# TGoldC/Motion-Planning-for-Autonomous-Driving-with-MPC

Hardware: AMD Instinct MI355X
Metric: MPC steps/sec (N=30, nx=6 nu=2) at batch=4096 (higher is better)
Workload: dtype f64; 1 GPU; N=30 nx=6 nu=2 bicycle lane-following, batch=4096/GPU, tol 1e-8; mode=converged, gpu=AMD Radeon Graphics

## Files before the change

### motion-planning-for-autonomous-driving-with-mpc_amd/csrc/mpc_solve_plan.h

```cpp
#pragma once
#include <algorithm>
#include <cctype>
#include <cstdlib>
#include <cstring>
#include <string>

#include "mpc_host_common.h"

namespace mpc {

struct Knobs {
    int pipeline, hybrid, hybrid_bx, hybrid_live, pipe_help, pipe_test_abort, pipe_xcd_mask;
    int rescue, rescue_wg, rescue_alone, loop_async, sync_spin, max_batch, friction_lb, bound_mask, big_wg, groups, poison;
    int timing;
    Knobs();
};
enum class KnobParse {
    ON,
    INT,
    FLAG,
    MASK,
    FRIC,
};
struct KnobDef { const char* name; int Knobs::*field; int dflt; KnobParse parse; };
inline constexpr KnobDef KNOBS[] = {
    {"pipeline", &Knobs::pipeline, 1, KnobParse::ON},           {"hybrid", &Knobs::hybrid, 1, KnobParse::INT},
    {"hybrid_bx", &Knobs::hybrid_bx, 0, KnobParse::INT},        {"hybrid_live", &Knobs::hybrid_live, -1, KnobParse::INT},
    {"pipe_help", &Knobs::pipe_help, -1, KnobParse::INT},       {"pipe_test_abort", &Knobs::pipe_test_abort, 0, KnobParse::FLAG},
    {"pipe_xcd_mask", &Knobs::pipe_xcd_mask, 0, KnobParse::MASK}, {"rescue", &Knobs::rescue, 1, KnobParse::ON},
    {"rescue_wg", &Knobs::rescue_wg, 1, KnobParse::INT},        {"rescue_alone", &Knobs::rescue_alone, 0, KnobParse::FLAG},
    {"loop_async", &Knobs::loop_async, 1, KnobParse::ON},       {"sync_spin", &Knobs::sync_spin, 1, KnobParse::ON},
    {"max_batch", &Knobs::max_batch, 0, KnobParse::INT},        {"friction_lb", &Knobs::friction_lb, 0, KnobParse::FRIC},
    {"bound_mask", &Knobs::bound_mask, 1, KnobParse::INT},      {"big_wg", &Knobs::big_wg, 0, KnobParse::FLAG},
    {"groups", &Knobs::groups, 0, KnobParse::INT},              {"poison", &Knobs::poison, 0, KnobParse::FLAG},
    {"timing", &Knobs::timing, 0, KnobParse::INT},
};
inline Knobs::Knobs() { for (const KnobDef& e : KNOBS) this->*e.field = e.dflt; }
inline const KnobDef* find_knob(const char* name) {
    for (const KnobDef& e : KNOBS) if (name && strcmp(name, e.name) == 0) return &e;
    return nullptr;
}
inline int set_knob(Knobs& k, const char* name, const char* value) {
    const KnobDef* e = find_knob(name);
    if (!e) return MPC_ERR_INVALID;
    int v = e->dflt;
    if (value) {
        const long iv = strtol(value, nullptr, 0);
        switch (e->parse) {
            case KnobParse::ON: v = value[0] != '0'; break;
            case KnobParse::INT: v = (int)iv; break;
            case KnobParse::FLAG: v = (value[0] == '\0' ? 1 : (int)iv) != 0; break;
            case KnobParse::MASK: v = (int)(uint32_t)strtoul(value, nullptr, 0); break;
            case KnobParse::FRIC: v = strcmp(value, "ipopt") == 0 ? 1 : strcmp(value, "nlp") == 0 ? 0 : (int)iv; break;
        }
    }
    k.*e->field = v;
    return MPC_OK;
}
// ... 19 lines not shown
              TIMING_WG_TRACE = 16;

constexpr int STAGE_MAX_THREADS = 512;
constexpr int MAX_GROUPS = 4;
constexpr int MAX_POLL_IT = 1024;
constexpr size_t LDS_MAX = 160 * 1024 - 1024;

#ifndef MPC_STAGE_STASH
#define MPC_STAGE_STASH 1
#endif
template <int NX> struct Stash {
    static constexpr int rows(bool has_ou) { return 4 * (NX + 2) + 2 * 3 + (has_ou ? 2 * 3 : 0) + 3 + 2 * NX; }
};

constexpr uint32_t REF_BOUND_VM = 0x33u;
constexpr uint32_t REF_DENSE_LO = 0x31u, REF_DENSE_HI = 0x33u;

constexpr int RIC_DEPTH = 4;
constexpr int RIC_DEPTH_F = 10;

constexpr uint32_t PIPE_X_STRIDE = 64;
enum PipeXcdWord : uint32_t { PX_ARRIVE = 0, PX_HEAD = 16, PX_TAIL = 32, PX_FINISHED = 48, PX_HO_TICKET = 56 };
constexpr uint32_t PIPE_ABORT = 8 * PIPE_X_STRIDE;
constexpr uint32_t HO_BUCKETS = 4;
enum PipeHeadWord : uint32_t {
    PH_ABORT = 0, PH_ROUNDS = 1,
    PH_STAT64 = 2,
    PH_STAGE_WORKERS = 12, PH_RIC_WORKERS = 13, PH_FAIL = 14,
    PH_WG = 16,
    PH_HELPED = 21, PH_FIN_TICKET = 22,
    PH_HO = 24,
    PH_DETAIL = 28,
    PH_WORDS = 32 };
enum PipeStat64 : uint32_t { P64_RIC_WAIT, P64_STAGE_WAIT, P64_STAGE_BUSY, P64_ITEMS };
enum WgStatWord : uint32_t { WGS_ROUNDS_MAX, WGS_ROUNDS, WGS_SWEEPS, WGS_INST_ROUNDS, WGS_RESCUED, WGS_WORDS };
constexpr uint32_t PIPE_STATS = PIPE_ABORT + PH_STAT64, PIPE_WG = PIPE_ABORT + PH_WG, PIPE_HO = PIPE_ABORT + PH_HO, PIPE_HDR = PIPE_ABORT + PH_WORDS;
struct CtlField { uint32_t at, words, align; };
template <size_t N> constexpr bool ctl_fields_ok(const CtlField (&f)[N], uint32_t size) {
    for (size_t i = 0; i < N; ++i) {
        if (f[i].at % f[i].align || f[i].at + f[i].words > size) return false;
        for (size_t j = 0; j < i; ++j) if (f[i].at < f[j].at + f[j].words && f[j].at < f[i].at + f[i].words) return false;
    }
    return true;
}
constexpr CtlField PIPE_HEAD_FIELDS[] = {{PH_ABORT, 1, 1}, {PH_ROUNDS, 1, 1}, {PH_STAT64, 8, 2}, {PH_STAGE_WORKERS, 1, 1}, {PH_RIC_WORKERS, 1, 1}, {PH_FAIL, 1, 1},
                                         {PH_WG, WGS_WORDS, 1}, {PH_HELPED, 1, 1}, {PH_FIN_TICKET, 1, 1}, {PH_HO, HO_BUCKETS, 1}, {PH_DETAIL, 4, 1}};
constexpr CtlField PIPE_XCD_FIELDS[] = {{PX_ARRIVE, 1, 1}, {PX_HEAD, 1, 1}, {PX_TAIL, 1, 1}, {PX_FINISHED, 1, 1}, {PX_HO_TICKET, 1, 1}};
static_assert(ctl_fields_ok(PIPE_HEAD_FIELDS, PH_WORDS) && PIPE_ABORT % 2 == 0 && PH_HO + HO_BUCKETS <= PH_DETAIL, "the head's fields are disjoint, inside it, the uint64 ones 8-byte aligned; the hand-over counters end in front of the abort details");
static_assert(ctl_fields_ok(PIPE_XCD_FIELDS, PIPE_X_STRIDE), "the fields of an XCD record are disjoint and inside it");
constexpr uint32_t pipe_slots_off(uint32_t ntiles) { return (PIPE_HDR + ntiles + 1u) & ~1u; }
constexpr size_t pipe_ctl_words(uint32_t ntiles, uint32_t cap) { return (size_t)pipe_slots_off(ntiles) + (size_t)16 * cap; }
constexpr int PIPE_MAX_TILES = 256;

constexpr size_t prestart_doubles(int NX, int S, int bx) { return (size_t)4 * S * (NX + 2) + (size_t)(3 * NX + 2) * S * bx + (size_t)4 * bx; }
template <int NX>
struct WgLds {
    static constexpr int PAD = Rec<NX>::SIZE > 64 ? Rec<NX>::SIZE : 64;
    static constexpr size_t doubles(int S, int bxw) { return (size_t)PAD + (size_t)Rec<NX>::SIZE * S * bxw + (size_t)2 * S * (NX + 2) + (size_t)16 * bxw + (size_t)64 * NX + (size_t)WgScl::SIZE * bxw; }
};

struct PlanState {
    int n_cu = 256;
    uint32_t xcd_mask = 0xFFu;
    bool ws_mailbox = false;
    bool pipe_disabled = false;
    bool resc_hint = false;
    int32_t B = 0;
    bool per_inst_obst = false;
    bool trace = false;
    bool in_rescue = false;
    bool async_loop = false;
};
struct SolvePlan {
    bool small_wg;
    int S, bx, threads, nblk, ntiles, G, stash_rows;
    size_t lds_bytes, lds_init, ric_lds;
    bool masked;
    int cap, chunk;
    bool polled;
    bool fused;
    size_t lds_pre, lds_start;
    bool res_path, pipe_path;
    int hyb_bx;
    bool resc_alone, hyb_ok;
    int hand;
    bool wg_resc;
    size_t wg_lds;
    int wg_grid;
    uint32_t xcd_mask;
    int n_xcd, tiles_x, cu_x, n_ric;
    uint32_t pipe_cap;
    bool pipe_help;
    int mbw_live;
    bool stage_timing, start_timing, wg_timing, wg_trace, pipe_timing, poison;
    size_t max_rows;
    bool mailbox;
    bool rescue;
    bool loop_async;
};

template <int NX>
SolvePlan plan_solve_nx(const HostProblem& hp, const Knobs& kn, const PlanState& st) {
    const mpc_problem_desc& d = hp.desc;
    const int B = st.B;
    SolvePlan pl{};
    const size_t Bp = ((size_t)B + 63) / 64 * 64;
    const int S = d.N + 1;
    pl.S = S;
    pl.ntiles = (int)(Bp / 64);
    const int ntiles = pl.ntiles;
    pl.small_wg = 4 * S <= 256 && !kn.big_wg;
// ... 24 lines not shown
    pl.fused = lds_red + pl.lds_pre + 16 + lds_in <= 78 * 1024 && d.N >= 1 && pl.small_wg;
    pl.lds_start = std::max(lds_red + pl.lds_pre + 16 + lds_in, pl.lds_init);

    auto wg_lds = [&](int bxw) {
        const size_t pre = prestart_doubles(NX, S, bxw) * sizeof(double);
        const size_t init = ((size_t)10 * bxw + (size_t)2 * S * (NX + 2) + (size_t)2 * NX * 64) * sizeof(double);
        return std::max(WgLds<NX>::doubles(S, bxw) * sizeof(double), bxw == 1 ? std::max(pre, init) : (size_t)0);
    };
    pl.rescue = kn.rescue && d.fixed_iters <= 0 && !st.trace && hp.has_ol && hp.ol_raw > 0.0;
    const bool resc_cond = pl.rescue && (kn.rescue_wg >= 2 || kn.rescue_alone || (kn.rescue_wg == 1 && st.resc_hint)) && !st.in_rescue;
    int hyb_bx = ((kn.hybrid_bx == 2 || (kn.hybrid_bx == 0 && B > 4 * st.n_cu)) && S * 2 <= 64) ? 2 : 1;
    if (kn.hybrid_bx == 0 && resc_cond && hyb_bx == 2 && (size_t)ntiles * 64 * 8 <= (size_t)4 * st.n_cu * 18) hyb_bx = 1;
    pl.resc_alone = kn.rescue_alone && kn.hybrid_bx == 0 && kn.hybrid_live < 0 && resc_cond && ntiles <= 128;
    if (pl.resc_alone || st.in_rescue) hyb_bx = 1;
    pl.hyb_bx = hyb_bx;
    pl.wg_resc = resc_cond && hyb_bx == 1;
    pl.wg_lds = wg_lds(hyb_bx);
    pl.mailbox = pl.small_wg && S <= 64 && kn.hybrid && d.fixed_iters <= 0 && kn.pipeline && !st.pipe_disabled;
    pl.hyb_ok = kn.hybrid && st.ws_mailbox && d.fixed_iters <= 0 && kn.pipeline && !st.pipe_disabled && G == 1 && pl.small_wg && S <= 64 &&
                pl.wg_lds <= LDS_MAX / 4 && !st.trace && !pl.stage_timing;
    int hand = 0;
    if (pl.hyb_ok) {
        const int base = std::min(64, 4 * st.n_cu * hyb_bx / std::max(1, ntiles));
        hand = base >= 64 ? base : std::max(base, std::min(50, base < 32 ? 7 * base / 4 : 3 * base / 2));
        if (hyb_bx == 1 && base < 64 && hand < 40) hand = 40;
        if ((size_t)ntiles * 64 * 8 <= (size_t)4 * st.n_cu * hyb_bx * (hyb_bx == 2 ? 9 : 18)) hand = 64;
        if (pl.resc_alone) hand = 64;
        if (kn.hybrid_live >= 0) hand = std::min(64, kn.hybrid_live);
    }
    pl.hand = hand;
    pl.res_path = pl.hyb_ok && (hand >= 64 || st.in_rescue);
    pl.xcd_mask = st.xcd_mask;
    if (kn.pipe_xcd_mask) {
        const uint32_t m = (uint32_t)kn.pipe_xcd_mask & st.xcd_mask;
        if (m) pl.xcd_mask = m;
    }
    pl.n_xcd = __builtin_popcount(pl.xcd_mask);
    pl.tiles_x = (ntiles + pl.n_xcd - 1) / pl.n_xcd;
    pl.cu_x = std::max(2, st.n_cu / pl.n_xcd);
    const int tiles_x = pl.tiles_x, cu_x = pl.cu_x;
    const int n_ric_base = std::max(1, cu_x / 4);
    const bool ric_per_tile = tiles_x > n_ric_base && tiles_x <= 3 * cu_x / 8 && (64 / bx) * tiles_x <= 5 * (cu_x - tiles_x) && S >= 24;
    pl.n_ric = std::min(ric_per_tile ? tiles_x : n_ric_base, tiles_x);
    const bool eligible = G == 1 && !st.trace && !pl.stage_timing && pl.small_wg && pl.threads >= 192 && pl.threads <= 256 &&
                          ntiles <= (d.fixed_iters > 0 ? 64 : PIPE_MAX_TILES) && (tiles_x + pl.n_ric - 1) / pl.n_ric <= 32 &&
                          std::max(pl.lds_bytes, pl.ric_lds) <= LDS_MAX;
    pl.pipe_path = !pl.res_path && eligible && !st.pipe_disabled && kn.pipeline;
    pl.pipe_cap = 1;
    while (pl.pipe_path && pl.pipe_cap < 2u * (64u / (uint32_t)bx) * (uint32_t)tiles_x) pl.pipe_cap <<= 1;
    pl.pipe_help = pl.pipe_path && pl.masked && (kn.pipe_help < 0 ? (64 / bx) * tiles_x > 3 * (cu_x - pl.n_ric) : kn.pipe_help != 0);
    pl.mbw_live = pl.pipe_path && hand > 0 ? std::min(63, hand + 16) : 0;
    pl.wg_grid = pl.res_path ? (B + hyb_bx - 1) / hyb_bx
               : pl.pipe_path && hand > 0 ? std::min((B + hyb_bx - 1) / hyb_bx, std::max(4 * st.n_cu, (int)((size_t)hand * ntiles + hyb_bx - 1) / hyb_bx)) : 0;
    pl.start_timing = (kn.timing & TIMING_START) && !st.async_loop && G == 1;
    pl.wg_timing = (kn.timing & TIMING_WG) && !st.async_loop;
    pl.wg_trace = (kn.timing & TIMING_WG_TRACE) && !st.async_loop && !st.in_rescue;
    pl.pipe_timing = (kn.timing & TIMING_PIPE) != 0;
    pl.poison = kn.poison && !st.in_rescue;

    const WsLayout w1 = ws_layout(d.N, NX, 64, pl.mailbox);
    pl.max_rows = (((size_t)1 << 32) - 1) / (w1.total * sizeof(double)) * 64;
    const bool pipe_shape = pl.small_wg && kn.pipeline && !st.pipe_disabled && kn.groups <= 0 && !pl.stage_timing && d.fixed_iters <= 0 &&
                            pl.threads >= 192 && pl.threads <= 256;
    if (pipe_shape) pl.max_rows = std::min(pl.max_rows, (size_t)PIPE_MAX_TILES * 64);
    if (kn.max_batch > 0) pl.max_rows = std::min(pl.max_rows, (size_t)(kn.max_batch + 63) / 64 * 64);
    pl.loop_async = d.fixed_iters <= 0 && kn.pipeline && !st.pipe_disabled && kn.loop_async && (size_t)B <= pl.max_rows;
    return pl;
}
inline SolvePlan plan_solve(const HostProblem& hp, const Knobs& kn, const PlanState& st) {
    return hp.desc.nx == 5 ? plan_solve_nx<5>(hp, kn, st) : plan_solve_nx<6>(hp, kn, st);
}

struct SolveIo {
    int32_t B = 0;
    const double *x0 = nullptr, *p = nullptr, *obst = nullptr;
    double *x_out = nullptr, *kkt = nullptr;
// ... 18 lines not shown
```

### motion-planning-for-autonomous-driving-with-mpc_amd/csrc/mpcgpu.hip

```cpp
#include <hip/hip_runtime.h>
#include <type_traits>

#include <algorithm>
#include <cctype>
#include <cstdio>
#include <cstdlib>
#include <cstring>
#include <new>
#include <string>
#include <vector>

#include "mpc_host_common.h"
#include "mpc_solve_plan.h"
#include "mpc_stamps.h"
#include "mpc_closed_loop.h"
#include "mpc_forces_qp.h"
#include "mpc_riccati_mfma.h"
#include "mpc_sens.h"

using namespace mpc;

namespace {

__device__ __forceinline__ void lds_barrier() {
// ... 280 lines not shown
    const uint32_t b0 = (blk + (uint32_t)P.tile0 * (64u / (uint32_t)P.bx)) * (uint32_t)P.bx;
    const unsigned long long bits = (!INIT && P.tile_mask != nullptr) ? P.tile_mask[b0 >> 6] : ~0ull;
    stage_block<NX, INIT, MAXT, VM>(P, n_mult, n_z, stash_rows, b0, bits, lds);
}

constexpr int32_t HO_IN_MB = 0x40000000;

template <int NCH>
__device__ __forceinline__ void wait_dma_behind(int stages_behind) {
    if (stages_behind >= 4 && 4 * NCH <= 63) asm volatile("s_waitcnt vmcnt(%0)" ::"n"(4 * NCH <= 63 ? 4 * NCH : 0) : "memory");
    else if (stages_behind >= 3 && 3 * NCH <= 63) asm volatile("s_waitcnt vmcnt(%0)" ::"n"(3 * NCH <= 63 ? 3 * NCH : 0) : "memory");
    else if (stages_behind >= 2) asm volatile("s_waitcnt vmcnt(%0)" ::"n"(2 * NCH) : "memory");
    else if (stages_behind == 1) asm volatile("s_waitcnt vmcnt(%0)" ::"n"(NCH) : "memory");
    else asm volatile("s_waitcnt vmcnt(0)" ::: "memory");
}

__device__ __forceinline__ void ho_lists(const PRef& P, const uint32_t bb, int32_t* ho_list, uint32_t* ho_count, const uint32_t* tile_word) {
#if defined(__HIP_DEVICE_COMPILE__)
    const int lane = threadIdx.x & 63;
    const bool active = (int)bb < P.B && (int32_t)MPC_U(P.ISC, (uint32_t)IS_STATUS) == ST_RUNNING;
    if (__ballot(active ? 1 : 0) == 0ull) return;
    const int32_t in_mb = (tile_word != nullptr && (__hip_atomic_load(tile_word + (bb >> 6), __ATOMIC_RELAXED, __HIP_MEMORY_SCOPE_AGENT) >> 31)) ? HO_IN_MB : 0;
    const double e0 = active ? (double)MPC_U(P.SC, (uint32_t)SC_E0) : 0.0;
    const int bucket = e0 >= 1e-3 ? 0 : e0 >= 1e-4 ? 1 : e0 >= 1e-5 ? 2 : 3;
    for (int q = 0; q < (int)HO_BUCKETS; ++q) {
        const unsigned long long mq = __ballot((active && bucket == q) ? 1 : 0);
        if (mq == 0ull) continue;
        uint32_t base = 0u;
        if (lane == 0) base = __hip_atomic_fetch_add(ho_count + q, (uint32_t)__popcll(mq), __ATOMIC_RELAXED, __HIP_MEMORY_SCOPE_AGENT);
        base = (uint32_t)__builtin_amdgcn_readfirstlane((int)base);
        if (active && bucket == q) ho_list[(uint32_t)q * (uint32_t)P.Bp + base + (uint32_t)__popcll(mq & ((1ull << lane) - 1ull))] = (int32_t)bb | in_mb;
    }
#endif
}

template <int NX>
__device__ __forceinline__ unsigned long long riccati_tile(const PRef& P, const uint32_t tile, char* smem, const bool stamp = true, const int handover_live = 0) {
#if defined(__HIP_DEVICE_COMPILE__)
    using D = Dim<NX>;
    constexpr int NS = D::NS;
    constexpr uint32_t BLK_BYTES = MPC_EV(D::NBLK) * 512u;
    constexpr int BLK_CHUNKS = (BLK_BYTES + 1023u) / 1024u;
    constexpr uint32_t SLOT = BLK_CHUNKS * 1024u;
    constexpr int KK_CHUNKS = (D::NKK * 512u + 1023u) / 1024u;
    constexpr int FWD_CHUNKS = KK_CHUNKS + 6;
    constexpr uint32_t FSLOT = FWD_CHUNKS * 1024u;
    static_assert(2 * BLK_CHUNKS <= 63 && RIC_DEPTH == 4 && 4 * FWD_CHUNKS <= 63 && RIC_DEPTH_F == 10, "vmcnt is a 6-bit counter");
    constexpr uint32_t RING_BYTES = (RIC_DEPTH * SLOT > RIC_DEPTH_F * FSLOT) ? RIC_DEPTH * SLOT : RIC_DEPTH_F * FSLOT;
    int* flag = reinterpret_cast<int*>(smem + RING_BYTES);
    const int wave = __builtin_amdgcn_readfirstlane((int)(threadIdx.x >> 6));
// ... 531 lines not shown
}

struct WgRescue { double ol_raw, relax; int32_t on; };
constexpr int RESC_LEVELS = 8;
__device__ __forceinline__ double resc_fraction(int q) { return q == 2 || q == 7 ? 1.0 : q == 4 ? 0.4 : q == 5 ? 0.7 : q == 6 ? 0.9 : 0.0; }
__device__ __forceinline__ bool resc_last(int q) { return q == 2 || q == 7; }

#if defined(__HIP_DEVICE_COMPILE__)
typedef const __attribute__((address_space(4))) Params* mpc_kernarg_params;
__device__ __forceinline__ mpc_kernarg_params wg_kernarg() {
    mpc_kernarg_params kp = (mpc_kernarg_params)__builtin_amdgcn_kernarg_segment_ptr();
    asm volatile("" : "+s"(kp));
    return kp;
}
__device__ __forceinline__ EmitDst wg_emit_dst() {
    const mpc_kernarg_params kp = wg_kernarg();
    return EmitDst{kp->x_out, kp->status_out, kp->iters_out, kp->kkt_out, kp->fail_count};
}
#else
inline EmitDst wg_emit_dst() { return EmitDst{}; }
#endif
template <int NX, int VAR, bool RESC>
__device__ __forceinline__ void solve_wg_body(const Params& Pk, const int n_mult, const int n_z, const int stash_rows, uint32_t* stats, const uint32_t* skip_if,
                                              const WgRescue& resc, unsigned long long* wtrace, const int32_t* list, const uint32_t* list_n) {
    PRef P(Pk);
#if defined(__HIP_DEVICE_COMPILE__)
    const bool emit_exit = RESC && resc.on && Pk.emit != 0;
    if (RESC && emit_exit) P.emit = 0;
    extern __shared__ __attribute__((aligned(16))) double lds[];
    __shared__ uint32_t sh_mask;
    __shared__ int sh_next[2];
    if (skip_if != nullptr && *skip_if != 0u) return;
    const double tol0 = P.tol;
    bool fresh = true;
    using D = Dim<NX>;
    using RC = Rec<NX>;
    const int bx = P.bx, t = threadIdx.x, N = P.N;
    const int lane = t;
    const uint32_t b0 = (blockIdx.x + (uint32_t)P.tile0 * (64u / (uint32_t)bx)) * (uint32_t)bx;
    int ib0 = (int)b0 < P.B ? (int)b0 : -1, ib1 = (bx > 1 && (int)b0 + 1 < P.B) ? (int)b0 + 1 : -1;
    uint32_t in_mb = 0u;
    if (list != nullptr) {
        uint32_t cnt[HO_BUCKETS], n = 0u;
#pragma unroll
        for (int q = 0; q < (int)HO_BUCKETS; ++q) { cnt[q] = list_n[q]; n += cnt[q]; }
        auto entry = [&](uint32_t v) -> int {
            if (v >= n) return -1;
#pragma unroll
            for (int q = 0; q < (int)HO_BUCKETS; ++q) { if (v < cnt[q]) return list[(uint32_t)q * (uint32_t)P.Bp + v]; v -= cnt[q]; }
            return -1;
        };
        const uint32_t G = gridDim.x;
        ib0 = lds_uniform(entry(blockIdx.x));
        ib1 = bx > 1 ? lds_uniform(entry(2u * G - 1u - blockIdx.x)) : -1;
        if (ib0 < 0) return;
        in_mb = ((ib0 & HO_IN_MB) ? 1u : 0u) | ((ib1 >= 0 && (ib1 & HO_IN_MB)) ? 2u : 0u);
        ib0 &= ~HO_IN_MB;
        if (ib1 >= 0) ib1 &= ~HO_IN_MB;
    }
    struct { int b, k, mb, bl; } c;
    c.k = t / bx;
    c.bl = t & (bx - 1);
    c.mb = (int)blockIdx.x * bx;
    c.b = c.bl ? ib1 : ib0;
    const bool valid = (c.k <= N) && (c.b >= 0) && (c.b < P.B);
    const mpc_lds_ptr recs = (mpc_lds_ptr)(lds_ptr_t)lds + WgLds<NX>::PAD;
    const mpc_lds_ptr dump = (mpc_lds_ptr)(lds_ptr_t)lds;
    double* const lds_bnd = lds + WgLds<NX>::PAD + (size_t)RC::SIZE * ((N + 1) * bx);
    double* const lds_c0 = lds_bnd + 2 * (N + 1) * D::NZ;
    double* const lds_r0 = lds_c0 + 8 * bx;
    double* const lds_rn = lds_r0 + 8 * bx;
    double* const lds_scl = lds_rn + 64 * NX;
    bool bounds_ok = false;
    double dl0 = 0.0, dl1 = 0.0;
    WgIo io{0u, 0u, lds_c0, lds_rn, lds_r0, lds_scl, true, false};
    const MfmaWords lane_words = mfma_lane_load<NX>(lane);
    uint32_t rounds = 0, sweeps = 0, inst_rounds = 0, prev_mask = 0u;
    const unsigned long long t_begin = wtrace ? wall_clock64() : 0ull;
    unsigned long long t_fresh = 0ull, t_round1 = 0ull;
    if (RESC && resc.on && t == 0 && ib0 >= 0 && ib0 < P.B) MPC_UB(P.ISC, (uint32_t)IS_RLEV, ib0) = 0;
    for (;;) {
        if (rounds == 0u && t < 64) {
            const int bb = t ? ib1 : ib0;
            const bool run = t < bx && bb >= 0 && bb < P.B && (list != nullptr || (int32_t)MPC_UB(P.ISC, (uint32_t)IS_STATUS, bb >= 0 ? bb : 0) == ST_RUNNING);
            const unsigned long long mk = __ballot(run ? 1 : 0);
            if (t == 0) sh_mask = (uint32_t)mk;
        }
        lds_barrier();
        const uint32_t mask = lds_uniform(sh_mask);
        if (Pk.emit != 0 && !emit_exit) {
            const uint32_t gone = prev_mask & ~mask;
            if (gone != 0u && valid && ((gone >> c.bl) & 1u)) {
                double z[MPC_EV(D::NZ)];
                ws_load_rows<D::NZ>(MPC_ROWS(MPC_KI(P.MZ, D::NZ, 0, e)), z);
                int st = 0, it = 0;
                double e0 = 0.0;
                if (c.k == 0) { st = (int32_t)MPC_S(P.ISC, IS_STATUS); it = (int32_t)MPC_S(P.ISC, IS_ITERS); e0 = MPC_S(P.SC, SC_E0); }
                emit_row<NX>(wg_emit_dst(), N, c.b, c.k, z, st, it, e0);
            }
            prev_mask = mask;
        }
        if (mask == 0u) {
            if (!RESC || !resc.on) break;
            if (t == 0) {
                const int bb = ib0;
                int next = -1, carry = 0;
                if (bb >= 0 && bb < P.B) {
                    const int st = (int32_t)MPC_UB(P.ISC, (uint32_t)IS_STATUS, bb), it = (int32_t)MPC_UB(P.ISC, (uint32_t)IS_ITERS, bb);
                    const int lev = (int32_t)MPC_UB(P.ISC, (uint32_t)IS_RLEV, bb);
                    const int q = lev & 0xFF;
                    int has_xs = (lev >> 8) & 1, first = lev & ~0x1FF;
                    int acc = (q == 0 ? 0 : (int32_t)MPC_UB(P.ISC, (uint32_t)IS_ITACC, bb)) + it;
                    if (q == 0) {
                        if (st == 0 || st == -7) { next = 1; first = (st == -7 ? 0x200 : 0) | (it << 16); if (stats != nullptr) atomicAdd(stats + WGS_RESCUED, 1u); }
                    } else {
                        if (st == 1) { carry = 1; has_xs = 1; }
                        if (!resc_last(q)) next = q + 1;
                        else if (st != 1 && q == 2) { next = 3; has_xs = 0; acc = first >> 16; }
                    }
                    if (next >= 0) {
                        MPC_UB(P.ISC, (uint32_t)IS_RLEV, bb) = next | (has_xs << 8) | first;
                        MPC_UB(P.ISC, (uint32_t)IS_ITACC, bb) = acc;
                        next |= has_xs << 8;
// ... 5 lines not shown
                sh_next[0] = next;
                sh_next[1] = carry;
            }
            lds_barrier();
            const int nx_lev = lds_uniform(sh_next[0]), carry = lds_uniform(sh_next[1]);
            lds_barrier();
            if (nx_lev <= -2) {
                const int code = -2 - nx_lev;
                const PRef Pc = P;
                wg_restore_first<NX>(Pc, (uint32_t)ib0, (code & 1) ? -7 : 0, code >> 1);
            }
            if (nx_lev < 0) break;
            const int q = nx_lev & 0xFF;
            const bool from_xs = (nx_lev >> 8) != 0;
            {
                const double lo = resc_fraction(q) * resc.ol_raw;
                P.ol = lo - resc.relax * fmax(1.0, fabs(lo));
                P.tol = resc_last(q) ? tol0 : fmax(tol0, 1e-4);
            }
            {
                const PRef Pc = P;
                wg_restart<NX>(Pc, n_mult, n_z, stash_rows, (uint32_t)ib0, lds, &sh_mask, carry != 0, from_xs, q == 1, rounds == 0u);
            }
            fresh = true;
            bounds_ok = false;
            io.have = false;
            continue;
        }
        ++rounds;
        inst_rounds += (uint32_t)__popc(mask);
        MPC_STAMP(P.DBG, blockIdx.x, WG_ROUND, t == 0 && rounds == 3u);
        const bool by_pipe = !RESC && valid && ((in_mb >> c.bl) & 1u) != 0u;
        if (fresh && valid && !by_pipe) {
            auto move = [&](auto cnt, auto from, auto to) {
                constexpr int CNT = decltype(cnt)::value;
                double v[MPC_EV(CNT)];
                ws_load_rows<CNT>(from, v);
                ws_store_rows<CNT>(to, v);
            };
            constexpr int NZ = D::NZ;
            move(std::integral_constant<int, NZ>{}, MPC_ROWS(MPC_K(P.Z, NZ, 0, e)), MPC_ROWS(MPC_KI(P.MZ, NZ, 0, e)));
            move(std::integral_constant<int, NZ>{}, MPC_ROWS(MPC_K(P.ZL, NZ, 0, e)), MPC_ROWS(MPC_KI(P.MZL, NZ, 0, e)));
            move(std::integral_constant<int, NZ>{}, MPC_ROWS(MPC_K(P.ZU, NZ, 0, e)), MPC_ROWS(MPC_KI(P.MZU, NZ, 0, e)));
            move(std::integral_constant<int, 4>{}, MPC_ROWS(MPC_K(P.SO, 3, 0, e)), MPC_ROWS(MPC_KI(P.MSO, 3, 0, e)));
            move(std::integral_constant<int, 4>{}, MPC_ROWS(MPC_K(P.NUO, 3, 0, e)), MPC_ROWS(MPC_KI(P.MNUO, 3, 0, e)));
            move(std::integral_constant<int, 4>{}, MPC_ROWS(MPC_K(P.ZLO, 3, 0, e)), MPC_ROWS(MPC_KI(P.MZLO, 3, 0, e)));
            move(std::integral_constant<int, 4>{}, MPC_ROWS(MPC_K(P.ZUO, 3, 0, e)), MPC_ROWS(MPC_KI(P.MZUO, 3, 0, e)));
            move(std::integral_constant<int, NX>{}, MPC_ROWS(MPC_K(P.LAM, NX, 0, e)), MPC_ROWS(MPC_KI(P.MLAM, NX, 0, e)));
        }
        if (fresh) {
            asm volatile("s_waitcnt vmcnt(0)" ::: "memory");
            __builtin_amdgcn_fence(__ATOMIC_ACQ_REL, "workgroup");
            asm volatile("s_waitcnt vmcnt(0)" ::: "memory");
        }
        const bool whole = fresh, tiled = fresh && !by_pipe;
        auto build_records = [&]() {
            if (valid && ((mask >> (t & (bx - 1))) & 1u)) {
                double blk[MPC_EV(D::NBLK)];
                if (tiled) ws_load_rows<D::NBLK>(MPC_ROWS(MPC_K(P.BLK, D::NBLK, 0, e)), blk);
                else ws_load_rows<D::NBLK>(MPC_ROWS(MPC_KI(P.MBLK, D::NBLK, 0, e)), blk);
                double hx0 = 0.0, hx1 = 0.0;
                if (c.k == 0) { hx0 = MPC_S(P.SC, SC_HUX0); hx1 = MPC_S(P.SC, SC_HUX1); }
                const mpc_lds_ptr r = recs + ((t & (bx - 1)) * (N + 1) + c.k) * RC::SIZE;
#pragma unroll
                for (int i = 0; i < D::NBLK; ++i) {
                    const bool kept = i < D::B_RUU || (i >= D::B_CN && i < D::B_CN + NX);
                    if (whole || !kept) r[RC::slot(i)] = (i >= D::B_CN && i < D::B_CN + NX) ? -blk[i] : blk[i];
                }
                r[RC::ZERO] = 0.0;
                r[RC::ONE] = 1.0;
                r[RC::DT] = P.dt;
                r[RC::HX] = hx0;
                r[RC::HX + 1] = hx1;
            }
        };
        if (fresh) {
            build_records();
            const int a0 = ib0 >= 0 ? ib0 : 0, a1 = ib1 >= 0 ? ib1 : a0;
            dl0 = lds_uniform((double)MPC_UB(P.SC, (uint32_t)SC_DLAST, a0));
            dl1 = lds_uniform((double)MPC_UB(P.SC, (uint32_t)SC_DLAST, a1));
            io.ill = ((int32_t)MPC_UB(P.ISC, (uint32_t)IS_ILL, a0) != 0 ? 1u : 0u) | ((bx > 1 && (int32_t)MPC_UB(P.ISC, (uint32_t)IS_ILL, a1) != 0) ? 2u : 0u);
            if (valid && c.k == 0) {
#pragma unroll
                for (int i = 0; i < NX; ++i) lds_c0[(t & (bx - 1)) * 8 + i] = MPC_S(P.SC, SC_C0 + i);
                double* q = lds_scl + c.bl * WgScl::SIZE;
                q[WgScl::MU] = MPC_S(P.SC, SC_MU); q[WgScl::TAU] = MPC_S(P.SC, SC_TAU); q[WgScl::DF] = MPC_S(P.SC, SC_DF); q[WgScl::THETA] = MPC_S(P.SC, SC_THETA);
                q[WgScl::FCOST] = MPC_S(P.SC, SC_FCOST); q[WgScl::LOGSUM] = MPC_S(P.SC, SC_LOGSUM); q[WgScl::THMAX] = MPC_S(P.SC, SC_THMAX);
                q[WgScl::THMIN] = MPC_S(P.SC, SC_THMIN); q[WgScl::A0LB] = MPC_S(P.SC, SC_A0LB); q[WgScl::A0UB] = MPC_S(P.SC, SC_A0UB);
                q[WgScl::STATUS] = (double)(int32_t)MPC_S(P.ISC, IS_STATUS); q[WgScl::NFILT] = (double)(int32_t)MPC_S(P.ISC, IS_NFILT);
                q[WgScl::ITERS] = (double)(int32_t)MPC_S(P.ISC, IS_ITERS); q[WgScl::CONV] = (double)(int32_t)MPC_S(P.ISC, IS_CONV);
                q[WgScl::FROW] = (double)(int32_t)MPC_S(P.ISC, IS_FROW); q[WgScl::HAVETH0] = (double)(int32_t)MPC_S(P.ISC, IS_HAVETH0);
            }
            {
                const bool f0 = ib0 >= 0 && t < 2 * FILTER_MAX, f1 = bx > 1 && ib1 >= 0 && t < 2 * FILTER_MAX;
                const double v0 = f0 ? (double)ws_ref3(P, P.FILT, 0u, (uint32_t)ib0, mpc_prow((uint32_t)t)) : 0.0;
                const double v1 = f1 ? (double)ws_ref3(P, P.FILT, 0u, (uint32_t)ib1, mpc_prow((uint32_t)t)) : 0.0;
                if (f0) lds_scl[WgScl::FILT + t] = v0;
                if (f1) lds_scl[WgScl::SIZE + WgScl::FILT + t] = v1;
            }
        }
        if (!bounds_ok) {
            const int nb = (N + 1) * D::NZ;
            fill_bounds<8>(P, lds_bnd, nb, t, 64);
            bounds_ok = true;
        }
        lds_barrier();
        if (wtrace != nullptr && fresh && t_fresh == 0ull) t_fresh = wall_clock64() - t_begin;
        fresh = false;
        MPC_STAMP(P.DBG, blockIdx.x, WG_RECORDS, t == 0 && rounds == 3u);
        MfmaWords lw = lane_words;
        asm volatile("" : "+v"(lw.w[0]), "+v"(lw.w[1]), "+v"(lw.w[2]), "+v"(lw.w[3]));
        MfmaLane<NX> m;
        mfma_lane_setup<NX>(m, lw, P.dt);
        constexpr uint32_t SVM = VAR == 2 ? REF_VM : 0xFFu;
        {
            auto inst_of = [&](int g, MfmaInst& in, double& x0) {
                in.inst = (uint32_t)(g ? ib1 : ib0);
                in.delta_last = g ? dl1 : dl0;
                in.sym_hint = ((io.ill >> g) & 1u) != 0u;
                x0 = 0.0;
                if ((lane & 3) == 0) {
                    if (m.Rb < NX) x0 = -lds_c0[g * 8 + m.Rb];
                    else if (m.Rb == 7) x0 = 1.0;
                }
            };
            io.fail = 0u;
            auto finish = [&](int g, bool ok, double delta) {
                const int bb = g ? ib1 : ib0;
                if (ok) { if (delta > 0.0) { if (g) dl1 = lds_uniform(delta); else dl0 = lds_uniform(delta); } }
                else io.fail |= 1u << g;
                if (lane != 0) return;
// ... 50 lines not shown
        if (rounds > 0u) ws_load_rows<D::NZ>(MPC_ROWS(MPC_KI(P.MZ, D::NZ, 0, e)), z);
        else ws_load_rows<D::NZ>(MPC_ROWS(MPC_K(P.Z, D::NZ, 0, e)), z);
        int st = 0, it = 0;
        double e0 = 0.0;
        if (c.k == 0) { st = (int32_t)MPC_S(P.ISC, IS_STATUS); it = (int32_t)MPC_S(P.ISC, IS_ITERS); e0 = MPC_S(P.SC, SC_E0); if (st == ST_RUNNING) st = 0; }
        emit_row<NX>(wg_emit_dst(), N, c.b, c.k, z, st, it, e0);
    }
    if (wtrace != nullptr && t == 0) {
        wtrace[blockIdx.x * 4 + 0] = t_begin;
        wtrace[blockIdx.x * 4 + 1] = wall_clock64();
        wtrace[blockIdx.x * 4 + 2] = rounds;
        wtrace[blockIdx.x * 4 + 3] = (unsigned long long)(inst_rounds & 0xFFFFu) | ((t_fresh & 0xFFFFFFull) << 16) | ((t_round1 & 0xFFFFFFull) << 40);
    }
    if (stats != nullptr && t == 0) {
        atomicMax(stats + WGS_ROUNDS_MAX, rounds);
        atomicAdd(stats + WGS_ROUNDS, rounds);
        atomicAdd(stats + WGS_SWEEPS, sweeps);
        atomicAdd(stats + WGS_INST_ROUNDS, inst_rounds);
    }
#endif
}
template <int NX, int VAR, bool RESC = false>
__global__ void __launch_bounds__(256) k_solve_wg(const Params Pk, const int n_mult, const int n_z, const int stash_rows, uint32_t* stats, const uint32_t* skip_if,
                                                                   const WgRescue resc, unsigned long long* wtrace, const int32_t* list, const uint32_t* list_n) {
    solve_wg_body<NX, VAR, RESC>(Pk, n_mult, n_z, stash_rows, stats, skip_if, resc, wtrace, list, list_n);
#if defined(__HIP_DEVICE_COMPILE__)
    if (threadIdx.x < 64) {
        const mpc_kernarg_params kp = wg_kernarg();
        uint32_t* const ctl = kp->fin_ctl;
        if (ctl == nullptr) return;
        uint32_t tk = 0u;
        if (threadIdx.x == 0) {
            asm volatile("s_waitcnt vmcnt(0)" ::: "memory");
            tk = __hip_atomic_fetch_add(ctl + PH_FIN_TICKET, 1u, __ATOMIC_RELAXED, __HIP_MEMORY_SCOPE_AGENT);
        }
        tk = (uint32_t)__builtin_amdgcn_readfirstlane((int)tk);
        if (tk == gridDim.x - 1u && threadIdx.x < PH_WORDS) {
            const uint32_t v = __hip_atomic_load(ctl + threadIdx.x, __ATOMIC_RELAXED, __HIP_MEMORY_SCOPE_AGENT);
            __hip_atomic_store(kp->fin_host + threadIdx.x, v, __ATOMIC_RELAXED, __HIP_MEMORY_SCOPE_SYSTEM);
        }
    }
#endif
}

template <int NX, class Src>
__device__ __forceinline__ void prestart_par_block(const PRef& P, const uint32_t b0, double* sm, const Src src) {
    constexpr bool WS = std::is_same<Src, PrestartFromWs>::value;
    constexpr int NZ = NX + 2;
// ... 1484 lines not shown
    return e;
}
template <int NX> static void launch_stage(const Solve& s, const Group& q, bool init) {
    Params Pg = s.P;
    Pg.tile0 = q.tile0;
    const auto kf = stage_kernel<NX>(s.pl.small_wg, init, s.pl.masked);
    hipLaunchKernelGGL(kf, dim3(q.nblk), dim3(s.pl.threads), init ? s.pl.lds_init : s.pl.lds_bytes, q.st, Pg, s.h->hp.n_mult, s.h->hp.n_z, s.pl.stash_rows);
}
template <int NX> static void launch_wg(Solve& s, const uint32_t* skip_if, const int32_t* list) {
    mpc_handle* h = s.h; const SolvePlan& pl = s.pl;
    if (pl.wg_trace) (void)stamp_rows(s.t_wtrace, s.n_wtrace = (s.io.B + pl.hyb_bx - 1) / pl.hyb_bx, s.stream, 4);
    Params Pw = s.P;
    Pw.bx = pl.hyb_bx;
    Pw.fin_ctl = h->async_loop ? nullptr : s.ctl + PIPE_ABORT; Pw.fin_host = h->h_pipe;
    if (skip_if != nullptr) Pw.DBG = nullptr;
    WgRescue rs{h->hp.ol_raw, BOUND_RELAX, 0};
    if (pl.wg_resc) {
        rs.on = 1;
        h->resc_ran = true;
        h->resc_in_kernel = list == nullptr;
    }
    const auto kf = wg_kernel<NX>(pl.masked, pl.wg_resc);
    hipLaunchKernelGGL(kf, dim3(pl.wg_grid), dim3(64), pl.wg_lds, s.stream, Pw, h->hp.n_mult, h->hp.n_z, pl.stash_rows, s.ctl + PIPE_WG, skip_if, rs, s.t_wtrace.as<unsigned long long>(), list,
                       list != nullptr ? (const uint32_t*)(s.ctl + PIPE_HO) : nullptr);
}
static void report_arrivals(const uint32_t* ctl, int ntiles, uint32_t items) {
    std::vector<uint32_t> sd((size_t)ntiles);
    if (hipMemcpy(sd.data(), ctl + PIPE_HDR, sd.size() * sizeof(uint32_t), hipMemcpyDeviceToHost) != hipSuccess) return;
    fprintf(stderr, "[mpcgpu]   arrivals per tile (items per tile and round: %u):", items);
    for (int q = 0; q < ntiles; ++q) fprintf(stderr, " %u%s", sd[q] & 0x7FFFFFFFu, (sd[q] >> 31) ? "r" : "");
    fprintf(stderr, "\n");
}
static void read_head(Solve& s) {
    mpc_handle* h = s.h; const uint32_t* hd = h->h_pipe;
    h->h_fail[FAIL_COUNT] = hd[PH_FAIL];
    if (h->resc_ran && !s.in_rescue) h->rescued_last = (int)hd[PH_WG + WGS_RESCUED];
    if (s.pl.res_path || s.pl.hand > 0) {
        h->res_prof[1] = 1; h->res_prof[2] = hd[PH_WG + WGS_ROUNDS_MAX]; h->res_prof[3] = s.pl.wg_grid;
        h->res_prof[4] = hd[PH_WG + WGS_ROUNDS]; h->res_prof[5] = hd[PH_WG + WGS_SWEEPS]; h->res_prof[6] = hd[PH_WG + WGS_INST_ROUNDS];
    }
    s.it = (int)hd[s.pl.pipe_path ? PH_ROUNDS : PH_WG + WGS_ROUNDS_MAX];
    if (s.pl.pipe_path) {
        const unsigned long long* st64 = reinterpret_cast<const unsigned long long*>(hd + PH_STAT64);
        h->pipe_prof[1] = 1; h->pipe_prof[2] = s.it;
        h->pipe_prof[3] = (double)st64[P64_RIC_WAIT] * 1e-5; h->pipe_prof[4] = (double)st64[P64_STAGE_WAIT] * 1e-5; h->pipe_prof[5] = (double)st64[P64_STAGE_BUSY] * 1e-5;
        h->pipe_prof[6] = (double)st64[P64_ITEMS]; h->pipe_prof[7] = (double)hd[PH_STAGE_WORKERS] + 1e-3 * (double)hd[PH_RIC_WORKERS];
    }
// ... 980 lines not shown
```

Measured before the change: 5.325 million MPC steps/s.

## Add persistent work-group refill of hand-over instances with finer error buckets

Adds an optional refill mode where a capped grid of work-group solvers takes a new hand-over instance from the bucketed list via an atomic ticket whenever a slot finishes, so the grid no longer needs one work-group per instance. Per-slot freshness bits let only the newly loaded slot reload its records. The hand-over buckets grow from 4 to 16, computed from the exponent bits of the initial error, and the wavefront-level bucket scatter now loops only over occupied buckets. Refill is off by default (wg_refill=0), so the default run mainly picks up the finer bucket ordering and the changed head layout.

```diff
diff --git a/motion-planning-for-autonomous-driving-with-mpc_amd/csrc/mpc_solve_plan.h b/motion-planning-for-autonomous-driving-with-mpc_amd/csrc/mpc_solve_plan.h
--- a/motion-planning-for-autonomous-driving-with-mpc_amd/csrc/mpc_solve_plan.h
+++ b/motion-planning-for-autonomous-driving-with-mpc_amd/csrc/mpc_solve_plan.h
@@ -12,6 +12,7 @@
 struct Knobs {
     int pipeline, hybrid, hybrid_bx, hybrid_live, pipe_help, pipe_test_abort, pipe_xcd_mask;
     int rescue, rescue_wg, rescue_alone, loop_async, sync_spin, max_batch, friction_lb, bound_mask, big_wg, groups, poison;
+    int hybrid_pct, wg_refill, wg_slots;
     int timing;
     Knobs();
 };
@@ -22,6 +23,7 @@
     MASK,
     FRIC,
 };
+constexpr int WG_REFILL_DEFAULT = 0;
 struct KnobDef { const char* name; int Knobs::*field; int dflt; KnobParse parse; };
 inline constexpr KnobDef KNOBS[] = {
     {"pipeline", &Knobs::pipeline, 1, KnobParse::ON},           {"hybrid", &Knobs::hybrid, 1, KnobParse::INT},
@@ -33,7 +35,8 @@
     {"max_batch", &Knobs::max_batch, 0, KnobParse::INT},        {"friction_lb", &Knobs::friction_lb, 0, KnobParse::FRIC},
     {"bound_mask", &Knobs::bound_mask, 1, KnobParse::INT},      {"big_wg", &Knobs::big_wg, 0, KnobParse::FLAG},
     {"groups", &Knobs::groups, 0, KnobParse::INT},              {"poison", &Knobs::poison, 0, KnobParse::FLAG},
-    {"timing", &Knobs::timing, 0, KnobParse::INT},
+    {"timing", &Knobs::timing, 0, KnobParse::INT},               {"hybrid_pct", &Knobs::hybrid_pct, -1, KnobParse::INT},
+    {"wg_refill", &Knobs::wg_refill, WG_REFILL_DEFAULT, KnobParse::INT}, {"wg_slots", &Knobs::wg_slots, 0, KnobParse::INT},
 };
 inline Knobs::Knobs() { for (const KnobDef& e : KNOBS) this->*e.field = e.dflt; }
 inline const KnobDef* find_knob(const char* name) {
@@ -99,16 +102,33 @@
 constexpr uint32_t PIPE_X_STRIDE = 64;
 enum PipeXcdWord : uint32_t { PX_ARRIVE = 0, PX_HEAD = 16, PX_TAIL = 32, PX_FINISHED = 48, PX_HO_TICKET = 56 };
 constexpr uint32_t PIPE_ABORT = 8 * PIPE_X_STRIDE;
-constexpr uint32_t HO_BUCKETS = 4;
+constexpr uint32_t HO_BUCKETS = 16;
+MPC_HD int ho_bucket_hi(const uint32_t h) {
+    const int32_t p = (int32_t)((h & 0x7FFFFFFFu) >> 9) - (1023 << 11);
+    if (p >= 0) return 0;
+    if (-p >= ((int32_t)HO_BUCKETS - 1) * 3402) return (int)HO_BUCKETS - 1;
+    const int32_t q = (int32_t)(((uint32_t)-p * 19731u) >> 26);
+    return q >= (int32_t)HO_BUCKETS - 2 ? (int)HO_BUCKETS - 1 : q + 1;
+}
+inline int ho_bucket(const double e) {
+    uint64_t u;
+    memcpy(&u, &e, sizeof u);
+    return ho_bucket_hi((uint32_t)(u >> 32));
+}
+inline int64_t ho_entry_slot(const uint32_t* cnt, uint32_t v, const size_t Bp) {
+    for (uint32_t q = 0; q < HO_BUCKETS; ++q) { if (v < cnt[q]) return (int64_t)((size_t)q * Bp + v); v -= cnt[q]; }
+    return -1;
+}
 enum PipeHeadWord : uint32_t {
     PH_ABORT = 0, PH_ROUNDS = 1,
     PH_STAT64 = 2,
     PH_STAGE_WORKERS = 12, PH_RIC_WORKERS = 13, PH_FAIL = 14,
     PH_WG = 16,
     PH_HELPED = 21, PH_FIN_TICKET = 22,
-    PH_HO = 24,
+    PH_WG_TICKET = 23,
     PH_DETAIL = 28,
-    PH_WORDS = 32 };
+    PH_HO = 32,
+    PH_WORDS = 48 };
 enum PipeStat64 : uint32_t { P64_RIC_WAIT, P64_STAGE_WAIT, P64_STAGE_BUSY, P64_ITEMS };
 enum WgStatWord : uint32_t { WGS_ROUNDS_MAX, WGS_ROUNDS, WGS_SWEEPS, WGS_INST_ROUNDS, WGS_RESCUED, WGS_WORDS };
 constexpr uint32_t PIPE_STATS = PIPE_ABORT + PH_STAT64, PIPE_WG = PIPE_ABORT + PH_WG, PIPE_HO = PIPE_ABORT + PH_HO, PIPE_HDR = PIPE_ABORT + PH_WORDS;
@@ -121,9 +141,9 @@
     return true;
 }
 constexpr CtlField PIPE_HEAD_FIELDS[] = {{PH_ABORT, 1, 1}, {PH_ROUNDS, 1, 1}, {PH_STAT64, 8, 2}, {PH_STAGE_WORKERS, 1, 1}, {PH_RIC_WORKERS, 1, 1}, {PH_FAIL, 1, 1},
-                                         {PH_WG, WGS_WORDS, 1}, {PH_HELPED, 1, 1}, {PH_FIN_TICKET, 1, 1}, {PH_HO, HO_BUCKETS, 1}, {PH_DETAIL, 4, 1}};
+                                         {PH_WG, WGS_WORDS, 1}, {PH_HELPED, 1, 1}, {PH_FIN_TICKET, 1, 1}, {PH_WG_TICKET, 1, 1}, {PH_HO, HO_BUCKETS, 1}, {PH_DETAIL, 4, 1}};
 constexpr CtlField PIPE_XCD_FIELDS[] = {{PX_ARRIVE, 1, 1}, {PX_HEAD, 1, 1}, {PX_TAIL, 1, 1}, {PX_FINISHED, 1, 1}, {PX_HO_TICKET, 1, 1}};
-static_assert(ctl_fields_ok(PIPE_HEAD_FIELDS, PH_WORDS) && PIPE_ABORT % 2 == 0 && PH_HO + HO_BUCKETS <= PH_DETAIL, "the head's fields are disjoint, inside it, the uint64 ones 8-byte aligned; the hand-over counters end in front of the abort details");
+static_assert(ctl_fields_ok(PIPE_HEAD_FIELDS, PH_WORDS) && PIPE_ABORT % 2 == 0 && PH_HO + HO_BUCKETS <= PH_WORDS && PH_WORDS <= 64, "the head's fields are disjoint, inside it, the uint64 ones 8-byte aligned; one wavefront copies the head to the host");
 static_assert(ctl_fields_ok(PIPE_XCD_FIELDS, PIPE_X_STRIDE), "the fields of an XCD record are disjoint and inside it");
 constexpr uint32_t pipe_slots_off(uint32_t ntiles) { return (PIPE_HDR + ntiles + 1u) & ~1u; }
 constexpr size_t pipe_ctl_words(uint32_t ntiles, uint32_t cap) { return (size_t)pipe_slots_off(ntiles) + (size_t)16 * cap; }
@@ -135,6 +155,8 @@
     static constexpr int PAD = Rec<NX>::SIZE > 64 ? Rec<NX>::SIZE : 64;
     static constexpr size_t doubles(int S, int bxw) { return (size_t)PAD + (size_t)Rec<NX>::SIZE * S * bxw + (size_t)2 * S * (NX + 2) + (size_t)16 * bxw + (size_t)64 * NX + (size_t)WgScl::SIZE * bxw; }
 };
+
+constexpr int HAND_CAP = 50;
 
 struct PlanState {
     int n_cu = 256;
@@ -164,6 +186,8 @@
     bool wg_resc;
     size_t wg_lds;
     int wg_grid;
+    bool wg_refill;
+    int wg_solo;
     uint32_t xcd_mask;
     int n_xcd, tiles_x, cu_x, n_ric;
     uint32_t pipe_cap;
@@ -234,10 +258,11 @@
     int hand = 0;
     if (pl.hyb_ok) {
         const int base = std::min(64, 4 * st.n_cu * hyb_bx / std::max(1, ntiles));
-        hand = base >= 64 ? base : std::max(base, std::min(50, base < 32 ? 7 * base / 4 : 3 * base / 2));
+        hand = base >= 64 ? base : std::max(base, std::min(HAND_CAP, base < 32 ? 7 * base / 4 : 3 * base / 2));
         if (hyb_bx == 1 && base < 64 && hand < 40) hand = 40;
         if ((size_t)ntiles * 64 * 8 <= (size_t)4 * st.n_cu * hyb_bx * (hyb_bx == 2 ? 9 : 18)) hand = 64;
         if (pl.resc_alone) hand = 64;
+        if (kn.hybrid_pct >= 0) hand = std::min(64, 64 * kn.hybrid_pct / 100);
         if (kn.hybrid_live >= 0) hand = std::min(64, kn.hybrid_live);
     }
     pl.hand = hand;
@@ -262,8 +287,12 @@
     while (pl.pipe_path && pl.pipe_cap < 2u * (64u / (uint32_t)bx) * (uint32_t)tiles_x) pl.pipe_cap <<= 1;
     pl.pipe_help = pl.pipe_path && pl.masked && (kn.pipe_help < 0 ? (64 / bx) * tiles_x > 3 * (cu_x - pl.n_ric) : kn.pipe_help != 0);
     pl.mbw_live = pl.pipe_path && hand > 0 ? std::min(63, hand + 16) : 0;
+    pl.wg_refill = pl.pipe_path && hand > 0 && kn.wg_refill != 0 && !pl.wg_resc;
+    const int wg_slots = kn.wg_slots > 0 ? kn.wg_slots : 4 * st.n_cu;
     pl.wg_grid = pl.res_path ? (B + hyb_bx - 1) / hyb_bx
+               : pl.wg_refill ? std::min((B + hyb_bx - 1) / hyb_bx, wg_slots)
                : pl.pipe_path && hand > 0 ? std::min((B + hyb_bx - 1) / hyb_bx, std::max(4 * st.n_cu, (int)((size_t)hand * ntiles + hyb_bx - 1) / hyb_bx)) : 0;
+    pl.wg_solo = pl.wg_refill ? pl.wg_grid / 8 : 0;
     pl.start_timing = (kn.timing & TIMING_START) && !st.async_loop && G == 1;
     pl.wg_timing = (kn.timing & TIMING_WG) && !st.async_loop;
     pl.wg_trace = (kn.timing & TIMING_WG_TRACE) && !st.async_loop && !st.in_rescue;
diff --git a/motion-planning-for-autonomous-driving-with-mpc_amd/csrc/mpcgpu.hip b/motion-planning-for-autonomous-driving-with-mpc_amd/csrc/mpcgpu.hip
--- a/motion-planning-for-autonomous-driving-with-mpc_amd/csrc/mpcgpu.hip
+++ b/motion-planning-for-autonomous-driving-with-mpc_amd/csrc/mpcgpu.hip
@@ -326,10 +326,12 @@
     if (__ballot(active ? 1 : 0) == 0ull) return;
     const int32_t in_mb = (tile_word != nullptr && (__hip_atomic_load(tile_word + (bb >> 6), __ATOMIC_RELAXED, __HIP_MEMORY_SCOPE_AGENT) >> 31)) ? HO_IN_MB : 0;
     const double e0 = active ? (double)MPC_U(P.SC, (uint32_t)SC_E0) : 0.0;
-    const int bucket = e0 >= 1e-3 ? 0 : e0 >= 1e-4 ? 1 : e0 >= 1e-5 ? 2 : 3;
-    for (int q = 0; q < (int)HO_BUCKETS; ++q) {
+    const int bucket = ho_bucket_hi((uint32_t)__double2hiint(e0));
+    unsigned long long todo = __ballot(active ? 1 : 0);
+    while (todo != 0ull) {
+        const int q = __builtin_amdgcn_readlane(bucket, (int)__builtin_ctzll(todo));
         const unsigned long long mq = __ballot((active && bucket == q) ? 1 : 0);
-        if (mq == 0ull) continue;
+        todo &= ~mq;
         uint32_t base = 0u;
         if (lane == 0) base = __hip_atomic_fetch_add(ho_count + q, (uint32_t)__popcll(mq), __ATOMIC_RELAXED, __HIP_MEMORY_SCOPE_AGENT);
         base = (uint32_t)__builtin_amdgcn_readfirstlane((int)base);
@@ -907,7 +909,7 @@
 #endif
 template <int NX, int VAR, bool RESC>
 __device__ __forceinline__ void solve_wg_body(const Params& Pk, const int n_mult, const int n_z, const int stash_rows, uint32_t* stats, const uint32_t* skip_if,
-                                              const WgRescue& resc, unsigned long long* wtrace, const int32_t* list, const uint32_t* list_n) {
+                                              const WgRescue& resc, unsigned long long* wtrace, const int32_t* list, uint32_t* list_n, const int solo) {
     PRef P(Pk);
 #if defined(__HIP_DEVICE_COMPILE__)
     const bool emit_exit = RESC && resc.on && Pk.emit != 0;
@@ -917,7 +919,7 @@
     __shared__ int sh_next[2];
     if (skip_if != nullptr && *skip_if != 0u) return;
     const double tol0 = P.tol;
-    bool fresh = true;
+    uint32_t fresh = 3u;
     using D = Dim<NX>;
     using RC = Rec<NX>;
     const int bx = P.bx, t = threadIdx.x, N = P.N;
@@ -925,19 +927,25 @@
     const uint32_t b0 = (blockIdx.x + (uint32_t)P.tile0 * (64u / (uint32_t)bx)) * (uint32_t)bx;
     int ib0 = (int)b0 < P.B ? (int)b0 : -1, ib1 = (bx > 1 && (int)b0 + 1 < P.B) ? (int)b0 + 1 : -1;
     uint32_t in_mb = 0u;
+    auto entries = [&](const uint32_t v0, const uint32_t v1, int& e0, int& e1) {
+        uint32_t lo = 0u;
+        int f0 = -1, f1 = -1;
+        uint32_t u0 = 0u, u1 = 0u;
+#pragma unroll
+        for (int q = 0; q < (int)HO_BUCKETS; ++q) {
+            const uint32_t hi = lo + lds_uniform(__hip_atomic_load(list_n + q, __ATOMIC_RELAXED, __HIP_MEMORY_SCOPE_AGENT));
+            if (v0 >= lo && v0 < hi) { f0 = q; u0 = v0 - lo; }
+            if (v1 >= lo && v1 < hi) { f1 = q; u1 = v1 - lo; }
+            lo = hi;
+        }
+        e0 = f0 >= 0 ? lds_uniform(list[(uint32_t)f0 * (uint32_t)P.Bp + u0]) : -1;
+        e1 = f1 >= 0 ? lds_uniform(list[(uint32_t)f1 * (uint32_t)P.Bp + u1]) : -1;
+    };
+    const bool refill = !RESC && list != nullptr && solo >= 0;
+    bool dry = !refill;
     if (list != nullptr) {
-        uint32_t cnt[HO_BUCKETS], n = 0u;
-#pragma unroll
-        for (int q = 0; q < (int)HO_BUCKETS; ++q) { cnt[q] = list_n[q]; n += cnt[q]; }
-        auto entry = [&](uint32_t v) -> int {
-            if (v >= n) return -1;
-#pragma unroll
-            for (int q = 0; q < (int)HO_BUCKETS; ++q) { if (v < cnt[q]) return list[(uint32_t)q * (uint32_t)P.Bp + v]; v -= cnt[q]; }
-            return -1;
-        };
         const uint32_t G = gridDim.x;
-        ib0 = lds_uniform(entry(blockIdx.x));
-        ib1 = bx > 1 ? lds_uniform(entry(2u * G - 1u - blockIdx.x)) : -1;
+        entries(blockIdx.x, bx > 1 ? 2u * G - 1u - blockIdx.x : ~0u, ib0, ib1);
         if (ib0 < 0) return;
         in_mb = ((ib0 & HO_IN_MB) ? 1u : 0u) | ((ib1 >= 0 && (ib1 & HO_IN_MB)) ? 2u : 0u);
         ib0 &= ~HO_IN_MB;
@@ -948,7 +956,7 @@
     c.bl = t & (bx - 1);
     c.mb = (int)blockIdx.x * bx;
     c.b = c.bl ? ib1 : ib0;
-    const bool valid = (c.k <= N) && (c.b >= 0) && (c.b < P.B);
+    bool valid = (c.k <= N) && (c.b >= 0) && (c.b < P.B);
     const mpc_lds_ptr recs = (mpc_lds_ptr)(lds_ptr_t)lds + WgLds<NX>::PAD;
     const mpc_lds_ptr dump = (mpc_lds_ptr)(lds_ptr_t)lds;
     double* const lds_bnd = lds + WgLds<NX>::PAD + (size_t)RC::SIZE * ((N + 1) * bx);
@@ -972,7 +980,7 @@
             if (t == 0) sh_mask = (uint32_t)mk;
         }
         lds_barrier();
-        const uint32_t mask = lds_uniform(sh_mask);
+        uint32_t mask = lds_uniform(sh_mask);
         if (Pk.emit != 0 && !emit_exit) {
             const uint32_t gone = prev_mask & ~mask;
             if (gone != 0u && valid && ((gone >> c.bl) & 1u)) {
@@ -984,6 +992,39 @@
                 emit_row<NX>(wg_emit_dst(), N, c.b, c.k, z, st, it, e0);
             }
             prev_mask = mask;
+        }
+        if (!RESC && !dry && rounds > 0u) {
+            const bool alone = (int)blockIdx.x < solo;
+            const uint32_t want = alone ? (mask == 0u ? 1u : 0u) : ~mask & ((1u << bx) - 1u);
+            if (want != 0u) {
+                const uint32_t n_want = (uint32_t)__popc(want);
+                uint32_t tk = 0u;
+                if (t == 0) tk = __hip_atomic_fetch_add(list_n + PH_WG_TICKET - PH_HO, n_want, __ATOMIC_RELAXED, __HIP_MEMORY_SCOPE_AGENT);
+                tk = lds_uniform(tk) + (uint32_t)bx * gridDim.x;
+                int e0, e1;
+                entries(tk, n_want > 1u ? tk + 1u : ~0u, e0, e1);
+                if (e0 < 0 || (n_want > 1u && e1 < 0)) dry = true;
+                const int g0 = (want & 1u) ? 0 : 1;
+                uint32_t got = 0u;
+                if (e0 >= 0) {
+                    if (g0 == 0) ib0 = e0 & ~HO_IN_MB; else ib1 = e0 & ~HO_IN_MB;
+                    in_mb = (in_mb & ~(1u << g0)) | ((e0 & HO_IN_MB) ? 1u << g0 : 0u);
+                    got |= 1u << g0;
+                }
+                if (e1 >= 0) {
+                    ib1 = e1 & ~HO_IN_MB;
+                    in_mb = (in_mb & ~2u) | ((e1 & HO_IN_MB) ? 2u : 0u);
+                    got |= 2u;
+                }
+                if (got != 0u) {
+                    c.b = c.bl ? ib1 : ib0;
+                    valid = (c.k <= N) && (c.b >= 0) && (c.b < P.B);
+                    fresh |= got;
+                    mask |= got;
+                    prev_mask = mask;
+                    io.have = false;
+                }
+            }
         }
         if (mask == 0u) {
             if (!RESC || !resc.on) break;
@@ -1035,7 +1076,7 @@
                 const PRef Pc = P;
                 wg_restart<NX>(Pc, n_mult, n_z, stash_rows, (uint32_t)ib0, lds, &sh_mask, carry != 0, from_xs, q == 1, rounds == 0u);
             }
-            fresh = true;
+            fresh = 3u;
             bounds_ok = false;
             io.have = false;
             continue;
@@ -1044,7 +1085,8 @@
         inst_rounds += (uint32_t)__popc(mask);
         MPC_STAMP(P.DBG, blockIdx.x, WG_ROUND, t == 0 && rounds == 3u);
         const bool by_pipe = !RESC && valid && ((in_mb >> c.bl) & 1u) != 0u;
-        if (fresh && valid && !by_pipe) {
+        const bool mine_fresh = ((fresh >> c.bl) & 1u) != 0u;
+        if (mine_fresh && valid && !by_pipe) {
             auto move = [&](auto cnt, auto from, auto to) {
                 constexpr int CNT = decltype(cnt)::value;
                 double v[MPC_EV(CNT)];
@@ -1066,9 +1108,9 @@
             __builtin_amdgcn_fence(__ATOMIC_ACQ_REL, "workgroup");
             asm volatile("s_waitcnt vmcnt(0)" ::: "memory");
         }
-        const bool whole = fresh, tiled = fresh && !by_pipe;
-        auto build_records = [&]() {
-            if (valid && ((mask >> (t & (bx - 1))) & 1u)) {
+        const bool whole = mine_fresh, tiled = mine_fresh && !by_pipe;
+        auto build_records = [&](const bool taken_over = false) {
+            if (valid && ((mask >> (t & (bx - 1))) & 1u) && (!taken_over || mine_fresh)) {
                 double blk[MPC_EV(D::NBLK)];
                 if (tiled) ws_load_rows<D::NBLK>(MPC_ROWS(MPC_K(P.BLK, D::NBLK, 0, e)), blk);
                 else ws_load_rows<D::NBLK>(MPC_ROWS(MPC_KI(P.MBLK, D::NBLK, 0, e)), blk);
@@ -1088,12 +1130,14 @@
             }
         };
         if (fresh) {
-            build_records();
+            build_records(true);
             const int a0 = ib0 >= 0 ? ib0 : 0, a1 = ib1 >= 0 ? ib1 : a0;
-            dl0 = lds_uniform((double)MPC_UB(P.SC, (uint32_t)SC_DLAST, a0));
-            dl1 = lds_uniform((double)MPC_UB(P.SC, (uint32_t)SC_DLAST, a1));
-            io.ill = ((int32_t)MPC_UB(P.ISC, (uint32_t)IS_ILL, a0) != 0 ? 1u : 0u) | ((bx > 1 && (int32_t)MPC_UB(P.ISC, (uint32_t)IS_ILL, a1) != 0) ? 2u : 0u);
-            if (valid && c.k == 0) {
+            const double d0 = lds_uniform((double)MPC_UB(P.SC, (uint32_t)SC_DLAST, a0)), d1 = lds_uniform((double)MPC_UB(P.SC, (uint32_t)SC_DLAST, a1));
+            if (fresh & 1u) dl0 = d0;
+            if (fresh & 2u) dl1 = d1;
+            const uint32_t ill = ((int32_t)MPC_UB(P.ISC, (uint32_t)IS_ILL, a0) != 0 ? 1u : 0u) | ((bx > 1 && (int32_t)MPC_UB(P.ISC, (uint32_t)IS_ILL, a1) != 0) ? 2u : 0u);
+            io.ill = (io.ill & ~fresh) | (ill & fresh);
+            if (valid && c.k == 0 && mine_fresh) {
 #pragma unroll
                 for (int i = 0; i < NX; ++i) lds_c0[(t & (bx - 1)) * 8 + i] = MPC_S(P.SC, SC_C0 + i);
                 double* q = lds_scl + c.bl * WgScl::SIZE;
@@ -1105,7 +1149,7 @@
                 q[WgScl::FROW] = (double)(int32_t)MPC_S(P.ISC, IS_FROW); q[WgScl::HAVETH0] = (double)(int32_t)MPC_S(P.ISC, IS_HAVETH0);
             }
             {
-                const bool f0 = ib0 >= 0 && t < 2 * FILTER_MAX, f1 = bx > 1 && ib1 >= 0 && t < 2 * FILTER_MAX;
+                const bool f0 = (fresh & 1u) && ib0 >= 0 && t < 2 * FILTER_MAX, f1 = (fresh & 2u) && bx > 1 && ib1 >= 0 && t < 2 * FILTER_MAX;
                 const double v0 = f0 ? (double)ws_ref3(P, P.FILT, 0u, (uint32_t)ib0, mpc_prow((uint32_t)t)) : 0.0;
                 const double v1 = f1 ? (double)ws_ref3(P, P.FILT, 0u, (uint32_t)ib1, mpc_prow((uint32_t)t)) : 0.0;
                 if (f0) lds_scl[WgScl::FILT + t] = v0;
@@ -1119,7 +1163,7 @@
         }
         lds_barrier();
         if (wtrace != nullptr && fresh && t_fresh == 0ull) t_fresh = wall_clock64() - t_begin;
-        fresh = false;
+        fresh = 0u;
         MPC_STAMP(P.DBG, blockIdx.x, WG_RECORDS, t == 0 && rounds == 3u);
         MfmaWords lw = lane_words;
         asm volatile("" : "+v"(lw.w[0]), "+v"(lw.w[1]), "+v"(lw.w[2]), "+v"(lw.w[3]));
@@ -1216,8 +1260,8 @@
 }
 template <int NX, int VAR, bool RESC = false>
 __global__ void __launch_bounds__(256) k_solve_wg(const Params Pk, const int n_mult, const int n_z, const int stash_rows, uint32_t* stats, const uint32_t* skip_if,
-                                                                   const WgRescue resc, unsigned long long* wtrace, const int32_t* list, const uint32_t* list_n) {
-    solve_wg_body<NX, VAR, RESC>(Pk, n_mult, n_z, stash_rows, stats, skip_if, resc, wtrace, list, list_n);
+                                                                   const WgRescue resc, unsigned long long* wtrace, const int32_t* list, uint32_t* list_n, const int solo) {
+    solve_wg_body<NX, VAR, RESC>(Pk, n_mult, n_z, stash_rows, stats, skip_if, resc, wtrace, list, list_n, solo);
 #if defined(__HIP_DEVICE_COMPILE__)
     if (threadIdx.x < 64) {
         const mpc_kernarg_params kp = wg_kernarg();
@@ -2748,7 +2792,7 @@
     }
     const auto kf = wg_kernel<NX>(pl.masked, pl.wg_resc);
     hipLaunchKernelGGL(kf, dim3(pl.wg_grid), dim3(64), pl.wg_lds, s.stream, Pw, h->hp.n_mult, h->hp.n_z, pl.stash_rows, s.ctl + PIPE_WG, skip_if, rs, s.t_wtrace.as<unsigned long long>(), list,
-                       list != nullptr ? (const uint32_t*)(s.ctl + PIPE_HO) : nullptr);
+                       list != nullptr ? s.ctl + PIPE_HO : (uint32_t*)nullptr, pl.wg_refill ? pl.wg_solo : -1);
 }
 static void report_arrivals(const uint32_t* ctl, int ntiles, uint32_t items) {
     std::vector<uint32_t> sd((size_t)ntiles);
```

New measurement: 5.139 million MPC steps/s. 3.5% lower.
